# gautam-sabnis/A-Divide-and-Conquer-Strategy-for-High-Dimensional-Bayesian-Factor-Models

Measured on AMD Instinct MI355X. Metric: Gibbs iters/sec (node) at p=20k,n=1k,g=64; cov-assembly MFMA util %, higher is better.
Workload: dtype f64; 1 GPU; c3: p=19968 (P=312 x g=64), n=1000, K=30 (k=1920), rho=0.5, thin=5, burnin=0 (assembly in timed region), asm_batch=96; global_batch=1000, parallelism=shards64/gpus1

## Files before the change

a-divide-and-conquer-strategy-for-high-dimensional-bayesian-factor-models_amd/csrc/dcfm.hip:

```cpp
#include "handle.h"
#include "resid.h"

static int dalloc(dcfm_handle *h, double **p, size_t n) {
    void *q = nullptr;
    if (n == 0) n = 1;
    hipError_t e = hipMalloc(&q, n * sizeof(double));
    if (e != hipSuccess)
        return fail(h, DCFM_ERR_ALLOC, "hipMalloc(%zu doubles) failed: %s", n, hipGetErrorString(e));
    e = hipMemset(q, 0, n * sizeof(double));
    if (e != hipSuccess) return fail(h, DCFM_ERR_HIP, "hipMemset failed: %s", hipGetErrorString(e));
    h->allocs.push_back(q);
    *p = static_cast<double *>(q);
    return DCFM_OK;
}

static int round_up(int a, int b) { return (a + b - 1) / b * b; }

static double *trace_row(dcfm_handle *h, int64_t t) {
    return h->trace + trace_scratch_doubles(h->d.G) + (size_t)t * h->d.G * 4;
}

static void collect_prof(dcfm_handle *h) {
    if (h->recs.empty()) return;
    sync_all(h);
// ... 353 lines not shown
    if (h->d.inject) {
        if (!h->dr.NZ) return fail(h, DCFM_ERR_INVALID, "INJECT_DRAWS set but no draws");
        if (first_iter < h->dr.first_iter || first_iter + n_iter > h->dr.first_iter + h->dr.n_iter)
            return fail(h, DCFM_ERR_INVALID, "iterations [%lld,%lld) not covered by injected draws",
                        (long long)first_iter, (long long)(first_iter + n_iter));
    }
    return DCFM_OK;
}

struct DeltaTau { const double *delta_in, *tau_in; double *delta_out, *tau_out; };
static DeltaTau delta_tau(const dcfm_handle *h) {
    const size_t nkg = (size_t)h->d.g * h->d.kp, in = h->cur * nkg, out = (1 - h->cur) * nkg;
    return {h->b.delta + in, h->b.tau + in, h->b.delta + out, h->b.tau + out};
}

static void iteration_done(dcfm_handle *h) {
    h->cur ^= 1;
    if (h->trace_n < h->trace_cap) {
        launch_trace(h->d, h->b, delta_tau(h).tau_in, h->trace, trace_row(h, h->trace_n), h->stream);
        h->trace_n += 1;
    }
}

static void loading_rows(dcfm_handle *h, const DrawsDev &dr, int64_t it, bool lamgen) {
    const Dims &d = h->d;
    const Bufs &b = h->b;
    hipStream_t s = h->stream;
    const bool exact = h->cfg.flags & DCFM_FLAG_EXACT_RESIDUAL;
    const double kappa_max = exact ? HUGE_VAL : (h->cfg.flags & DCFM_FLAG_GUARD_ALL) ? 0.0 : KAPPA_IDENTITY_MAX;
    {
        KTimer t(h, DCFM_K_LAMBDA, s);
        launch_lambda(d, b, dr, it, delta_tau(h).tau_in, h->plam_valid ? b.Plam : nullptr, s, lamgen, kappa_max);
    }
    if (exact) {
        KTimer t(h, DCFM_K_RESID, s);
        launch_resid(d, b, dr, it, s, lamgen);
    } else if (d.kp != KP) {
        KTimer t(h, DCFM_K_RESID, s);
        launch_resid_flagged(d, b, dr, it, s);
    }
    h->plam_valid = false;
}

static int save_sample(dcfm_handle *h, int64_t it) {
    if (it % h->cfg.thin != 0 || it <= h->cfg.burnin) return DCFM_OK;
    const Bufs &b = h->b;
    hipStream_t s = h->stream;
    if (h->batch == 0 && h->asm_pending[h->lb]) {
        HIPC(h, hipStreamWaitEvent(s, h->e_free[h->lb], 0));
        h->asm_pending[h->lb] = false;
    }
    {
        KTimer t(h, DCFM_K_SAVE, s);
        launch_save(h->d, b, b.Lb[h->lb], b.wsum[h->lb], h->batch, s, b.wslot[h->lb], h->B);
        if (h->probe_n < h->probe_cap) launch_probes(h->d, b, h->probes, h->probe_n++, s);
        if (h->prec_n < h->prec_cap) launch_precision(h->d, b, h->prec, h->prec_n++, s);
    }
    HIPC(h, hipGetLastError());
    h->batch += 1;
    h->saved += 1;
    if (h->batch == h->B) TRY(flush_batch(h));
    return DCFM_OK;
}

struct FusedSchedule {
    dcfm_handle *h;
    const Dims &d;
    const Bufs &b;
    hipStream_t s;
    bool delta_pending = false;
    const DrawsDev &draws() const { return d.inject ? h->dr : h->gen[0]; }

    int step(int64_t it) {
        const DrawsDev &dr = draws();
        const bool lamgen = !d.inject;
        { KTimer t(h, DCFM_K_WPASS, s); launch_wcol(d, b, dr, it, true, delta_pending, true, ++h->wc_ops, s, lamgen); }
        if (d.coll) {
            { KTimer t(h, DCFM_K_XRED, s); launch_xred(d, b, s); }
            KTimer t(h, DCFM_K_COMM, s);
            TRY(coll_allgather(h, CH_MAIN, b.sloc, b.msg_all, (size_t)d.xstride, s));
        }
        {
            KTimer t(h, DCFM_K_XDRAW, s);
            if (d.coll) launch_xdraw_mr(d, b, dr, it, ++h->xm_ops, s);
            else launch_xdraw(d, b, dr, it, s, true);
        }
        {
            KTimer t(h, DCFM_K_CPASS, s);
            const DeltaTau dt = delta_tau(h);
            if (delta_pending) launch_cpass(d, b, s, dr, dt.delta_in, dt.tau_in, dt.delta_out, dt.tau_out, it - 1);
            else launch_cpass(d, b, s);
        }
        HIPC(h, hipGetLastError());
        if (delta_pending) iteration_done(h);
        loading_rows(h, dr, it, lamgen);
        delta_pending = true;
        return DCFM_OK;
    }

    int tail(int64_t last_iter) {
        if (!delta_pending) return DCFM_OK;
        KTimer t(h, DCFM_K_DELTA, s);
        launch_wcol(d, b, h->dr, last_iter, false, true, false, 0, s);
        if (d.coll) TRY(coll_allgather(h, CH_MAIN, b.sloc, b.msg_all, (size_t)d.xstride, s));
        const DeltaTau dt = delta_tau(h);
        launch_delta(d, b, draws(), last_iter, dt.delta_in, dt.tau_in, dt.delta_out, dt.tau_out, s);
        HIPC(h, hipGetLastError());
        iteration_done(h);
        return DCFM_OK;
    }
};

struct DrawBatches {
    dcfm_handle *h;
    int64_t end_iter;
    int64_t batch0, batch_n = 0;
    int slot = -1;
    int generate(int64_t b0, int busy) {
// ... 59 lines not shown
        if (!d.inject) TRY(gen.acquire(it));
        const DrawsDev &dr = d.inject ? h->dr : h->gen[gen.slot];
        HIPC(h, hipStreamWaitEvent(ss, h->e_lam, 0));
        { KTimer t(h, DCFM_K_PREP, ss); launch_prep(d, b, ss); }
        HIPC(h, hipEventRecord(h->e_prep, ss));
        { KTimer t(h, DCFM_K_XCHOL, ss); launch_asum(d, b, ss); }
        if (d.coll) {
            KTimer t(h, DCFM_K_COMM, ss);
            TRY(coll_allgather(h, CH_SIDE, b.xa, b.xa_all, KW * KW, ss));
        }
        { KTimer t(h, DCFM_K_XCHOL, ss); launch_xchol(d, b, ss); }
        HIPC(h, hipEventRecord(h->e_xchol, ss));
        { KTimer t(h, DCFM_K_WPASS, s);  launch_wpass(d, b, s); }
        HIPC(h, hipStreamWaitEvent(s, h->e_prep, 0));
        { KTimer t(h, DCFM_K_ZDRAW, s);  launch_zdraw(d, b, dr, it, s); }
        { KTimer t(h, DCFM_K_XRED, s);   launch_xred(d, b, s); }
        if (d.coll) {
            KTimer t(h, DCFM_K_COMM, s);
            TRY(coll_allgather(h, CH_MAIN, b.xin, b.xall, (size_t)d.NP * KW, s));
        }
        HIPC(h, hipStreamWaitEvent(s, h->e_xchol, 0));
        { KTimer t(h, DCFM_K_XDRAW, s); launch_xdraw(d, b, dr, it, s, false); }
        { KTimer t(h, DCFM_K_CPASS, s); launch_cpass(d, b, s); }
        loading_rows(h, dr, it, false);
        HIPC(h, hipEventRecord(h->e_lam, s));
        { KTimer t(h, DCFM_K_COLSUM, s); launch_colsum(d, b, s); }
        if (d.coll) {
            KTimer t(h, DCFM_K_COMM, s);
            TRY(coll_allgather(h, CH_MAIN, b.sloc, b.sall, (size_t)d.G * KW, s));
        }
        {
            KTimer t(h, DCFM_K_DELTA, s);
            const DeltaTau dt = delta_tau(h);
            launch_delta(d, b, dr, it, dt.delta_in, dt.tau_in, dt.delta_out, dt.tau_out, s);
        }
        if (!d.inject) TRY(gen.release(it));
        iteration_done(h);
        return DCFM_OK;
    }
};

int dcfm_run(dcfm_handle *h, int64_t first_iter, int64_t n_iter) {
    TRY(check_run_args(h, first_iter, n_iter));
    HIPC(h, hipSetDevice(h->cfg.device));
    hipStream_t s = h->stream;
    const int64_t end_iter = first_iter + n_iter;
    FusedSchedule fused{h, h->d, h->b, s};
// ... 126 lines not shown
```

a-divide-and-conquer-strategy-for-high-dimensional-bayesian-factor-models_amd/csrc/dcfm_internal.h:

```cpp
#pragma once
#include <hip/hip_runtime.h>
#include <stdint.h>

namespace dcfm {

constexpr int KP = 32;
constexpr int KP_MAX = 128;
constexpr int padded_width(int K) { return K <= 32 ? 32 : (K <= 64 ? 64 : 128); }
constexpr int ASM_TILE = 128;
__host__ __device__ constexpr int etile(int nbw, int Kc, int I) { return Kc * nbw - Kc * (Kc - 1) / 2 + (I - Kc); }
__host__ __device__ constexpr int etile_index(int nbw, int R, int Cc) {
    return (2 * etile(nbw, R >> 4, Cc >> 4) + ((R & 15) >> 3)) * 128 + 2 * ((Cc & 15) + 16 * (R & 3)) +
           (((R & 15) >> 2) & 1);
}
constexpr int ASM_KC = 16;
inline int cdiv(int a, int b) { return (a + b - 1) / b; }

struct Dims {
    int n, P, g, K, G;
    int NP, PP;
    int shard0;
    int nranks, rank;
    int coll;
    int p;
    int kp;
    double rho, sr, s1r;
    double as_, bs, df, ad1, bd1, ad2, bd2;
    uint64_t seed;
    int inject;
    int sgap, xstride;
};

struct DrawsDev {
    const double *NZ, *NX, *NL, *Gpsi, *Gdelta, *Gps;
    int64_t first_iter, n_iter;
};

struct LamDraws { const double *NL, *Gpsi, *Gps; };
#ifndef DCFM_LAM_GEN_BLOCKS
#define DCFM_LAM_GEN_BLOCKS 160
#endif
constexpr int LAM_GEN_THREADS = 256, LAM_GEN_BLOCKS = DCFM_LAM_GEN_BLOCKS;
struct LamGen { double *NL, *Gpsi, *Gps; int n_ps, n_psi, n_all, b_total; };
inline int lam_gen_doubles(const Dims &d) { return 2 * d.G * d.P * d.K + d.G * d.P; }
inline LamGen lam_gen_plan(const Dims &d, double *base) {
    const int T = LAM_GEN_THREADS, GP = d.G * d.P;
    LamGen g;
    g.NL = base;
    g.Gpsi = base + (size_t)GP * d.K;
    g.Gps = base + 2 * (size_t)GP * d.K;
    g.n_ps = GP;
    g.n_psi = GP + GP * d.K;
    g.n_all = g.n_psi + GP * ((d.K + 1) / 2);
    const int full = (g.n_all + T - 1) / T;
    g.b_total = full < LAM_GEN_BLOCKS ? full : LAM_GEN_BLOCKS;
    return g;
}

struct Bufs {
    double *Y, *yy, *Lam, *omega, *ps, *psi, *Plam, *X, *Z, *delta, *tau;
    double *ldraw;
// ... 66 lines not shown
}
__host__ __device__ inline long long win_off(long long c, long long c0, long long R0, long long R1) {
    const long long na = (c < R0 ? c : R0) - c0;
    const long long b0 = c0 > R0 ? c0 : R0, b1 = c < R1 ? c : R1;
    return (na > 0 ? na : 0) * (R1 - R0) + (b1 > b0 ? b1 - b0 : 0) * R1;
}

void launch_prep(const Dims &d, const Bufs &b, hipStream_t s);
void launch_wpass(const Dims &d, const Bufs &b, hipStream_t s);
void launch_zdraw(const Dims &d, const Bufs &b, const DrawsDev &dr, int64_t iter, hipStream_t s);
void launch_xred(const Dims &d, const Bufs &b, hipStream_t s);
void launch_wcol(const Dims &d, const Bufs &b, const DrawsDev &dr, int64_t iter, bool ops, bool colsum, bool wpass,
                 unsigned long long ops_epoch, hipStream_t s, bool lamgen = false);
void launch_xdraw_mr(const Dims &d, const Bufs &b, const DrawsDev &dr, int64_t iter, unsigned long long xm_epoch,
                     hipStream_t s);
void launch_asum(const Dims &d, const Bufs &b, hipStream_t s);
void launch_xchol(const Dims &d, const Bufs &b, hipStream_t s);
void launch_xdraw(const Dims &d, const Bufs &b, const DrawsDev &dr, int64_t iter, hipStream_t s,
                  bool from_shards = false);
void launch_cpass(const Dims &d, const Bufs &b, hipStream_t s, const DrawsDev &dr = DrawsDev{},
                  const double *delta_in = nullptr, const double *tau_in = nullptr, double *delta_out = nullptr,
                  double *tau_out = nullptr, int64_t delta_iter = 0);
void launch_lambda(const Dims &d, const Bufs &b, const DrawsDev &dr, int64_t iter,
                   const double *tau_cur, const double *plam_src, hipStream_t s, bool gen, double kappa_max);
void launch_colsum(const Dims &d, const Bufs &b, hipStream_t s);
void launch_resid(const Dims &d, const Bufs &b, const DrawsDev &dr, int64_t iter, hipStream_t s, bool gen);
void launch_resid_flagged(const Dims &d, const Bufs &b, const DrawsDev &dr, int64_t iter, hipStream_t s);
void launch_delta(const Dims &d, const Bufs &b, const DrawsDev &dr, int64_t iter,
                  const double *delta_in, const double *tau_in, double *delta_out,
                  double *tau_out, hipStream_t s);
void launch_save(const Dims &d, const Bufs &b, double *Lb, double *wsum, int slot, hipStream_t s,
                 double *wslot = nullptr, int B = 0);
void launch_assemble(const Dims &d, const Bufs &b, const double *Lb, const double *wsum, int kext,
                     double inv_eff, hipStream_t s);
void launch_assemble_m2(const Dims &d, const Bufs &b, const double *Lb, const double *wslot, int nslots, int B,
                        double inv_eff, hipStream_t s);
void launch_sigma_pack(const double *S, const double *S2, int which, double rs, int p, int T0, int T1, int c0,
                       int nc, double *out, hipStream_t s);
void launch_sigma_unpack(const double *recv, int p, int c0, int nc, const int *Tb, const long long *base,
                         int nranks, double *out, hipStream_t s);
void launch_eta(const Dims &d, const Bufs &b, double *eta_out, hipStream_t s);
int sigma_err_splits(int p);
void launch_sigma_err(const double *S, int p, const double *U, int R, const double *sdiag, const double *v,
                      int T0, int T1, bool first, double *y, double *fro, double *tru, double *out,
                      hipStream_t s);
size_t sigma_apply_scratch(int T0, int T1, int nv);
void launch_sigma_apply(const double *S, int p, int T0, int T1, const double *V, int nv, double *scratch, double *Y,
// ... 28 lines not shown
```

a-divide-and-conquer-strategy-for-high-dimensional-bayesian-factor-models_amd/csrc/kernels.hip:

```cpp
#include "dcfm_internal.h"
#include "philox.h"
#include "linalg.h"
#include "handoff.h"
#include "wstamp.h"
#include "zx_ops.h"
#include "ypass.h"
#include "draws.h"
#include "zdraw.h"
#include "delta.h"
#include "lambda.h"

#include <algorithm>

namespace dcfm {

__global__ __launch_bounds__(256) void k_prep(Dims d, const double *__restrict__ Lam,
                                              const double *__restrict__ omega,
                                              double *__restrict__ A, double *__restrict__ ZM) {
    __shared__ double smem[PREP_SMEM];
    prep_shard(d, Lam, omega, A, ZM, blockIdx.x, smem);
}

template <int KW>
__global__ __launch_bounds__(256) void k_wpass(Dims d, const double *__restrict__ Y,
// ... 27 lines not shown
    const int e = blockIdx.x * 256 + threadIdx.x;
    const int kk = d.kp * d.kp;
    if (e >= kk) return;
    xa[e] = tree_sum(A + e, d.G, (size_t)kk);
}

__global__ __launch_bounds__(256) void k_xchol(Dims d, const double *__restrict__ xa_all,
                                               double *__restrict__ XM) {
    __shared__ double smem[XCHOL_SMEM];
    for (int e = threadIdx.x; e < KP * KP; e += 256) {
        xprec_store(d, smem, e, tree_sum(xa_all + e, d.nranks, (size_t)d.xstride));
    }
    __syncthreads();
    xchol_factor(d, XM, smem);
}

__device__ __forceinline__ void xdraw_chunks(int nsrc, int &nch, int &chunk) {
    chunk = 1;
    while (nsrc / chunk > 4 && (nsrc / chunk) % 2 == 0) chunk *= 2;
    nch = nsrc / chunk;
    if (nch > 4) { nch = 1; chunk = nsrc; }
}
constexpr int XD_ROWS = 4;
constexpr int XD_SMEM = (2 * KP * (KP + 1) + 4 * 4 * 64 * 2) > XCHOL_SMEM ? (2 * KP * (KP + 1) + 4 * 4 * 64 * 2)
                                                                          : XCHOL_SMEM;
__global__ __launch_bounds__(1024) void k_xdraw(Dims d, const double *__restrict__ src, int nsrc, size_t sstride,
                                                double *__restrict__ XM,
                                                double *__restrict__ X, DrawsDev dr, int64_t iter, int xroles,
                                                const double *__restrict__ xa, unsigned long long *xm_ctr,
                                                unsigned long long xm_target) {
    __shared__ double smem[XD_SMEM];
    int blk = blockIdx.x;
    if (xroles & 1) {
        if (blk == 0) {
            for (int e = threadIdx.x; e < KP * KP; e += 1024)
                xprec_store(d, smem, e, d.nranks > 1 ? tree_sum(xa + e, d.nranks, (size_t)d.xstride) : xa[e]);
            __syncthreads();
            xchol_factor<true>(d, XM, smem);
            signal_count(xm_ctr);
            return;
        }
        blk -= 1;
    }
    double (*Ms)[KP][KP + 1] = reinterpret_cast<double (*)[KP][KP + 1]>(smem);
    d2 (*part)[4][64] = reinterpret_cast<d2 (*)[4][64]>(smem + 2 * KP * (KP + 1));
    const int lane = threadIdx.x & 63, w = threadIdx.x >> 6, c = lane & 15, q = lane >> 4;
    const int tw = w & 3, sw = w >> 2;
    const int i0 = blk * XD_ROWS, i = i0 + c;
    const bool live = c < XD_ROWS && i < d.n;
    const size_t stride = sstride;
    int nch, chunk;
    xdraw_chunks(nsrc, nch, chunk);
    d2 sv[4], ev[4];
    if (w == 0 && d.inject) {
        const double *nx = dr.NX + ((size_t)(iter - dr.first_iter) * d.n + (live ? i : 0)) * d.K;
#pragma unroll
        for (int t = 0; t < 4; ++t) {
            const int kk = 8 * t + 2 * q;
            ev[t].x = (live && kk < d.K) ? nx[kk] : 0.0;
            ev[t].y = (live && kk + 1 < d.K) ? nx[kk + 1] : 0.0;
        }
    } else if (w == 0) {
        const Rng rng(d.seed);
#pragma unroll
        for (int t = 0; t < 4; ++t) {
            const int kk = 8 * t + 2 * q;
            double n0 = 0.0, n1 = 0.0;
            if (live && kk < d.K) rng.normal2(SITE_X, 0u, (uint32_t)i, (uint32_t)(4 * t + q), (uint32_t)iter, n0, n1);
            ev[t].x = n0;
            ev[t].y = (kk + 1 < d.K) ? n1 : 0.0;
        }
    }
    double xmv[2] = {0.0, 0.0};
    if (!(xroles & 1)) {
#pragma unroll
        for (int u = 0; u < 2; ++u) xmv[u] = XM[threadIdx.x + 1024 * u];
    }
    if (sw < nch) {
        if (chunk >= 2) {
            constexpr int NPART = 16 / XD_ROWS;
            const int np = (chunk & (chunk - 1)) ? 1 : (chunk < NPART ? chunk : NPART), per = chunk / np;
            const int rr = c % XD_ROWS, h = c / XD_ROWS;
            const bool rl = i0 + rr < d.n && h < np;
            const double *p = src + (size_t)(sw * chunk + (h < np ? h : 0) * per) * stride +
                              (size_t)(i0 + rr < d.n ? i0 + rr : i0) * KP + 8 * tw + 2 * q;
            d2 v = rl ? tree_sum_f<d2, 8, 10>(per, [&](int rk) { return *reinterpret_cast<const d2 *>(p + (size_t)rk * stride); })
                      : d2{0.0, 0.0};
            for (int o = 1; o < np; o <<= 1) {
                d2 u;
                u.x = __shfl_down(v.x, o * XD_ROWS, 16);
                u.y = __shfl_down(v.y, o * XD_ROWS, 16);
                v.x = v.x + u.x;
                v.y = v.y + u.y;
            }
            part[sw][tw][lane] = h == 0 ? v : d2{0.0, 0.0};
        } else {
            const double *p = src + (size_t)sw * chunk * stride + (size_t)(live ? i : i0) * KP + 8 * tw + 2 * q;
            part[sw][tw][lane] = live ? *reinterpret_cast<const d2 *>(p) : d2{0.0, 0.0};
        }
    }
    if (xroles & 1) {
        wait_count(xm_ctr, xm_target);
#pragma unroll
        for (int u = 0; u < 2; ++u) xmv[u] = ld_agent(XM + threadIdx.x + 1024 * u);
    }
#pragma unroll
    for (int u = 0; u < 2; ++u) {
        const int e = threadIdx.x + 1024 * u;
        const int mat = e / (KP * KP), rem = e % (KP * KP);
        Ms[mat][rem / KP][rem % KP] = xmv[u];
    }
    __syncthreads();
    if (w > 0) return;
#pragma unroll
    for (int t = 0; t < 4; ++t) {
        TreeSum<d2, 3> ts;
        for (int k = 0; k < nch; ++k) ts.push(part[k][t][lane]);
        sv[t] = ts.total();
    }
    d4 ax[2];
    ax[0] = ax[1] = d4{0.0, 0.0, 0.0, 0.0};
#pragma unroll
    for (int t = 0; t < 4; ++t)
#pragma unroll
        for (int e = 0; e < 2; ++e) {
            const int kk = 8 * t + 2 * q + e;
            const double se = e ? sv[t].y : sv[t].x, ee = e ? ev[t].y : ev[t].x;
#pragma unroll
            for (int mt = 0; mt < 2; ++mt) {
                ax[mt] = mfma16x16x4(Ms[0][16 * mt + c][kk], se, ax[mt]);
                ax[mt] = mfma16x16x4(Ms[1][16 * mt + c][kk], ee, ax[mt]);
            }
        }
    if (!live) return;
    double *Xr = X + (size_t)i * KP;
#pragma unroll
// ... 332 lines not shown
    da.delta_in = delta_in; da.tau_in = tau_in; da.delta_out = delta_out; da.tau_out = tau_out;
    da.iter = delta_iter;
    const int ndel = (delta_in && d.kp == KP) ? cdiv(d.g, CP_WAVES) : 0;
    switch (d.kp) {
    case 32:
        if (grid.x < 128)
            hipLaunchKernelGGL((k_cpass<32, true>), dim3(2 * grid.x + ndel), dim3(64 * CP_WAVES), 0, s, d, b.Y,
                               b.X, b.Z, b.C, b.E, dr, b.sall, da, ndel);
        else
            hipLaunchKernelGGL((k_cpass<32, false>), dim3(grid.x + ndel), dim3(64 * CP_WAVES), 0, s, d, b.Y, b.X,
                               b.Z, b.C, b.E, dr, b.sall, da, ndel);
        break;
    case 64:
        launch_eta(d, b, b.W, s);
        hipLaunchKernelGGL(k_cpass<64>, grid, dim3(256), 0, s, d, b.Y, b.W, b.Z, b.C, b.E, dr, b.sall, da, 0);
        break;
    default:
        launch_eta(d, b, b.W, s);
        hipLaunchKernelGGL(k_cpass<128>, grid, dim3(256), 0, s, d, b.Y, b.W, b.Z, b.C, b.E, dr, b.sall, da, 0);
        break;
    }
}
void launch_lambda(const Dims &d, const Bufs &b, const DrawsDev &dr, int64_t iter,
                   const double *tau_cur, const double *plam_src, hipStream_t s, bool gen, double kappa_max) {
    if (d.kp != KP) return wide::launch_lambda(d, b, dr, iter, tau_cur, plam_src, s, kappa_max);
    const LamDraws ld = lam_draws_at(d, b, dr, iter, gen);
    const dim3 grid(cdiv(d.P, LAM_ROWS), d.G);
#define LAUNCH_LAM(KE)                                                                                       \
    hipLaunchKernelGGL(k_lambda<KE>, grid, dim3(64), 0, s, d, b.C, b.E, b.yy, tau_cur, b.Lam, b.psi, plam_src, \
                       b.ps, b.omega, b.cpart, ld, b.Y, b.X, b.Z, kappa_max)
    if (d.K <= 8) LAUNCH_LAM(8);
    else if (d.K <= 16) LAUNCH_LAM(16);
    else if (d.K <= 20) LAUNCH_LAM(20);
    else if (d.K <= 24) LAUNCH_LAM(24);
    else if (d.K <= 30) LAUNCH_LAM(30);
    else LAUNCH_LAM(32);
#undef LAUNCH_LAM
}
void launch_colsum(const Dims &d, const Bufs &b, hipStream_t s) {
    const dim3 grid(d.G, d.kp / 32);
    switch (d.kp) {
    case 32: hipLaunchKernelGGL(k_colsum<32>, grid, dim3(256), 0, s, d, b.cpart, b.sloc); break;
    case 64: hipLaunchKernelGGL(k_colsum<64>, grid, dim3(256), 0, s, d, b.cpart, b.sloc); break;
    default: hipLaunchKernelGGL(k_colsum<128>, grid, dim3(256), 0, s, d, b.cpart, b.sloc); break;
    }
}
void launch_delta(const Dims &d, const Bufs &b, const DrawsDev &dr, int64_t iter,
                  const double *delta_in, const double *tau_in, double *delta_out, double *tau_out,
                  hipStream_t s) {
    if (d.kp != KP) return wide::launch_delta(d, b, dr, iter, delta_in, tau_in, delta_out, tau_out, s);
    hipLaunchKernelGGL(k_delta, dim3(d.g), dim3(64), 0, s, d, b.sall, delta_in, tau_in, delta_out,
                       tau_out, dr, iter);
}
// ... 51 lines not shown
```

a-divide-and-conquer-strategy-for-high-dimensional-bayesian-factor-models_amd/csrc/lambda.h:

```cpp
#pragma once
#include "dcfm_internal.h"
#include "philox.h"
#include "linalg.h"
#include "resid.h"

namespace dcfm {

#ifndef DCFM_LAM_ILP
#define DCFM_LAM_ILP 4
#endif
constexpr int LAM_ILP = DCFM_LAM_ILP;
__device__ __forceinline__ void lam_draws(const Dims &d, const LamGen &lg, int64_t iter, int gtid, int gthreads) {
    const Rng rng(d.seed);
    const uint32_t it = (uint32_t)iter;
    const int kp2 = (d.K + 1) / 2;
    for (int x = gtid; x < lg.n_ps; x += gthreads) {
        const int m = x / d.P, j = x - m * d.P;
        lg.Gps[x] = rng.gamma(d.as_ + 0.5 * d.n, SITE_PS, (uint32_t)(d.shard0 + m), (uint32_t)j, 0u, it);
    }
    const double sh = d.df * 0.5 + 0.5;
    const int npsi = lg.n_psi - lg.n_ps;
    if (sh == 1.0 || sh == 2.0) {
        for (int y0 = gtid; y0 < npsi; y0 += LAM_ILP * gthreads) {
            double u[LAM_ILP];
// ... 59 lines not shown

struct LamPiv { double i00, i11, l10, v0, v1, t10; };
__device__ __forceinline__ LamPiv lam_pivots(d2 pk, d2 pk1, d2 bb) {
    LamPiv p;
    const double a = pk.x, bq = pk1.x, c2 = pk1.y;
    p.i00 = rsqrt_f64(a);
    p.l10 = bq * p.i00;
    const double d11 = c2 - p.l10 * p.l10;
    p.i11 = rsqrt_f64(d11);
    p.v0 = bb.x * p.i00;
    p.v1 = (bb.y - p.l10 * p.v0) * p.i11;
    p.t10 = p.l10 * p.i11;
    return p;
}

template <int KE>
__global__ __launch_bounds__(64) __attribute__((amdgpu_waves_per_eu(2))) void k_lambda(Dims d, const double *__restrict__ C, const double *__restrict__ E,
                                               const double *__restrict__ yy, const double *__restrict__ tau_cur,
                                               double *__restrict__ Lam, double *__restrict__ psi,
                                               const double *__restrict__ plam_src, double *__restrict__ ps,
                                               double *__restrict__ omega, double *__restrict__ cpart,
                                               LamDraws ld, const double *__restrict__ Y,
                                               const double *__restrict__ X, const double *__restrict__ Z,
                                               double kappa_max) {
    static_assert(KE % 2 == 0 && KE >= 2 && KE <= KP, "even factor width");
    constexpr int NB = (KE + 7) / 8;
    constexpr int LSN = 2 * LAM_ROWS * (KP + 1) * 2, BSN = 2 * LAM_ROWS * (KP + 2), VSN = LAM_ROWS * (KP + 2);
    constexpr int EP = KP + 2;
    static_assert(KP * EP <= LSN + BSN, "E staging fits the image area");
    __shared__ __attribute__((aligned(16))) double SM[LSN + BSN + 2 * VSN + KP];
    double(*LS)[LAM_ROWS][KP + 1][2] = reinterpret_cast<double(*)[LAM_ROWS][KP + 1][2]>(SM);
    double(*BS)[LAM_ROWS][KP + 2] = reinterpret_cast<double(*)[LAM_ROWS][KP + 2]>(SM + LSN);
    double *Vs = SM + LSN + BSN, *Is = Vs + VSN;
    double *Dg = SM + LSN + BSN + 2 * VSN;
    double *Es = SM;
    const int m = blockIdx.y, mg = d.shard0 + m;
    const int lane = threadIdx.x, grp = lane >> 3, l = lane & 7;
    Vs += grp * (KP + 2);
    Is += grp * (KP + 2);
    const int j0 = blockIdx.x * LAM_ROWS;
    const int j = j0 + grp;
    const bool valid = j < d.P;
    const int jj = valid ? j : 0;
    const uint32_t rowoff = (uint32_t)(m * d.PP + jj) * KP, toff = (uint32_t)mg * KP;
    bool rv[4];
#pragma unroll
    for (int b = 0; b < 4; ++b) rv[b] = valid && l + 8 * b < d.K;
// ... 228 lines not shown
#pragma unroll
    for (int b = 0; b < NB; ++b) {
        const double e = Dg[l + 8 * b < KE ? l + 8 * b : 0];
        sabs = (rv[b] && e > 0.0) ? fma(fabs(x[b]), e * __builtin_amdgcn_rsq(e), sabs) : sabs;
    }
    cs = fmax(cs, dpp8_d<0xB1>(cs));
    cs = fmax(cs, dpp8_d<0x4E>(cs));
    cs = fmax(cs, dpp8_d<0x141>(cs));
    double mag = valid ? (fma(cs + 1.0, ww, px) + 2.0 * wva) * ipsj : 0.0;
    sabs = rowsum8(sabs);
    mag = rowsum8(mag);
    const double SS = yyj + contrib;
    const bool reject = ss_identity_reject(yyj, SS, mag, sabs, kappa_max);
    const bool exact = __any(valid && reject);
    if (valid) {
#pragma unroll
        for (int b = 0; b < 4; ++b) {
            const int r = l + 8 * b;
            const double ps_b = rv[b] ? (1.0 / (d.df * 0.5 + 0.5 * (x[b] * x[b] * tv[b]))) * G[b] : 0.0;
            Lam[rowoff + r] = x[b];
            cpart[rowoff + r] = ps_b * (x[b] * x[b]);
            if (rv[b]) psi[rowoff + r] = ps_b;
        }
    }
    if (exact) {
        double(*Lm)[KP + 1] = reinterpret_cast<double(*)[KP + 1]>(SM);
#pragma unroll
        for (int b = 0; b < 4; ++b) Lm[grp][l + 8 * b] = x[b];
        __builtin_amdgcn_wave_barrier();
        const int cc = lane & 15;
        const double gps_c = ld.Gps[(uint32_t)(m * d.P) + (j0 + cc < d.P && cc < LAM_ROWS ? j0 + cc : 0)];
        resid_rows8(d, Y, X, Z, Lm, gps_c, m, j0, lane, ps, omega);
    } else if (valid && l == 0) {
        ps_omega_store(d, SS, Gps, ps, omega, (uint32_t)(m * d.PP + j));
    }
}

}
```

a-divide-and-conquer-strategy-for-high-dimensional-bayesian-factor-models_amd/csrc/linalg.h:

```cpp
#pragma once
#include <hip/hip_runtime.h>
#include "dcfm_internal.h"
#include "philox.h"

#include <type_traits>
#include <utility>

namespace dcfm {

typedef double d4 __attribute__((ext_vector_type(4)));
typedef double d2 __attribute__((ext_vector_type(2)));

__device__ __forceinline__ d4 mfma16x16x4(double a, double b, d4 c) {
    return __builtin_amdgcn_mfma_f64_16x16x4f64(a, b, c, 0, 0, 0);
}
__device__ __forceinline__ d4 mfma16x16x4_na(double a, double b, d4 c) {
    return __builtin_amdgcn_mfma_f64_16x16x4f64(a, b, c, 0, 0, 1);
}

__device__ __forceinline__ double readlane_d(double x, int l) {
    const int lo = __builtin_amdgcn_readlane(__double2loint(x), l);
    const int hi = __builtin_amdgcn_readlane(__double2hiint(x), l);
    return __hiloint2double(hi, lo);
}
// ... 24 lines not shown
            if (open) {
                if ((i >> Q) & 1) {
                    v = s[Q] + v;
                } else {
                    s[Q] = v;
                    open = false;
                }
            }
        });
        ++i;
    }
    __device__ __forceinline__ T total() const {
        T acc{};
        bool have = false;
        static_for<L>([&](auto Q) {
            if ((i >> Q) & 1) {
                acc = have ? s[Q] + acc : s[Q];
                have = true;
            }
        });
        return acc;
    }
};
template <class T, int B = 8, int L = TREE_LEVELS, class F>
__device__ __forceinline__ T tree_sum_f(int n, F &&load) {
    TreeSum<T, L> ts;
    for (int k = 0; k < n; k += B) {
        T v[B];
        static_for<B>([&](auto U) { if (k + U < n) v[U] = load(k + U); });
        static_for<B>([&](auto U) { if (k + U < n) ts.push(v[U]); });
    }
    return ts.total();
}
__device__ __forceinline__ double tree_sum(const double *__restrict__ src, int n, size_t stride) {
    return tree_sum_f<double>(n, [&](int k) { return src[(size_t)k * stride]; });
}

__device__ __forceinline__ double rsqrt_f64(double x) {
    double y = __builtin_amdgcn_rsq(x);
#pragma unroll
    for (int it = 0; it < 2; ++it) {
        const double e = fma(-x * y, y, 1.0);
        y = fma(0.5 * y, e, y);
    }
    return y;
}
// ... 353 lines not shown
```

a-divide-and-conquer-strategy-for-high-dimensional-bayesian-factor-models_amd/csrc/resid.h:

```cpp
#pragma once
#include "dcfm_internal.h"
#include "linalg.h"

namespace dcfm {

__device__ __forceinline__ void ps_omega_store(const Dims &d, double SS, double Gps, double *ps, double *omega,
                                               size_t at) {
    const double psn = (1.0 / (d.bs + 0.5 * SS)) * Gps;
    ps[at] = psn;
    omega[at] = 1.0 / psn;
}

#ifndef DCFM_KAPPA_MAX
#define DCFM_KAPPA_MAX 1e3
#endif
constexpr double KAPPA_IDENTITY_MAX = DCFM_KAPPA_MAX;
__device__ __forceinline__ bool ss_identity_reject(double yy, double SS, double mag, double sabs, double kappa_max) {
    const double rt = 1.01 * (yy * __builtin_amdgcn_rsq(yy) + sabs);
    const double num = fmax(rt * rt, 1.01 * (yy + mag));
    return !(SS > 0.0 && num <= kappa_max * SS);
}

__device__ __forceinline__ d2 eta_pair(const Dims &d, d2 x, d2 z) {
    return d2{eta_of(d.sr, d.s1r, x.x, z.x), eta_of(d.sr, d.s1r, x.y, z.y)};
}
template <int NT, int NH, class EtaAt>
__device__ __forceinline__ void resid_chunk(const d4 (&y)[NH], EtaAt eta_at, const d2 (&lb)[NH][NT], int row0, int n,
                                            double (&ss)[NH]) {
    d4 acc[NH];
#pragma unroll
    for (int h = 0; h < NH; ++h) acc[h] = y[h];
#pragma unroll
    for (int t = 0; t < NT; ++t) {
// ... 2 lines not shown
        for (int h = 0; h < NH; ++h) acc[h] = mfma16x16x4_na(e.x, lb[h][t].x, acc[h]);
#pragma unroll
        for (int h = 0; h < NH; ++h) acc[h] = mfma16x16x4_na(e.y, lb[h][t].y, acc[h]);
    }
#pragma unroll
    for (int h = 0; h < NH; ++h)
#pragma unroll
        for (int v = 0; v < 4; ++v)
            ss[h] = (row0 + 4 * v < n) ? fma(acc[h][v], acc[h][v], ss[h]) : ss[h];
}
template <int NH>
__device__ __forceinline__ void resid_lanesum(double (&ss)[NH]) {
#pragma unroll
    for (int h = 0; h < NH; ++h) {
        ss[h] += xor16_d(ss[h]);
        ss[h] += xor32_d(ss[h]);
    }
}

constexpr int LAM_ROWS = 8;
__device__ __forceinline__ void resid_rows8(const Dims &d, const double *__restrict__ Y,
                                            const double *__restrict__ X, const double *__restrict__ Z,
                                            const double (*Lm)[KP + 1], double Gps_c, int m, int j0, int lane,
                                            double *__restrict__ ps, double *__restrict__ omega) {
    constexpr int NT = KP / 8;
    const int c = lane & 15, q = lane >> 4;
    const bool col = c < LAM_ROWS && j0 + c < d.P;
    d2 lb[1][NT];
#pragma unroll
    for (int t = 0; t < NT; ++t) {
        lb[0][t].x = col ? Lm[c][8 * t + 2 * q] : 0.0;
        lb[0][t].y = col ? Lm[c][8 * t + 2 * q + 1] : 0.0;
    }
    const double *Ym = Y + (size_t)m * d.NP * d.PP + (col ? j0 + c : 0);
    const double *Zm = Z + (size_t)m * d.NP * KP + 2 * q;
    double ss[1] = {0.0};
    for (int i0 = 0; i0 < d.NP; i0 += 16) {
        d4 y[1];
#pragma unroll
        for (int v = 0; v < 4; ++v) y[0][v] = col ? Ym[(size_t)(i0 + q + 4 * v) * d.PP] : 0.0;
        const double *xr = X + (size_t)(i0 + c) * KP + 2 * q, *zr = Zm + (size_t)(i0 + c) * KP;
        resid_chunk(y, [&](int t) {
            return eta_pair(d, *reinterpret_cast<const d2 *>(xr + 8 * t), *reinterpret_cast<const d2 *>(zr + 8 * t));
        }, lb, i0 + q, d.n, ss);
    }
    resid_lanesum(ss);
    if (q == 0 && col) ps_omega_store(d, ss[0], Gps_c, ps, omega, (uint32_t)(m * d.PP + j0 + c));
}

template <int KW>
__device__ __forceinline__ void resid_tile(const Dims &d, const double *__restrict__ Y, const double *__restrict__ X,
                                           const double *__restrict__ Z, const double *__restrict__ Lam,
                                           const double *__restrict__ Gps, double *__restrict__ ps,
                                           double *__restrict__ omega, int m, int j0, double (*red)[32]) {
    constexpr int NT = KW / 8;
    const int lane = threadIdx.x & 63, w = threadIdx.x >> 6, c = lane & 15, q = lane >> 4;
    const double *Ym = Y + (size_t)m * d.NP * d.PP;
    const double *Zm = Z + (size_t)m * d.NP * KW;
    d2 lb[2][NT];
#pragma unroll
    for (int h = 0; h < 2; ++h)
#pragma unroll
        for (int t = 0; t < NT; ++t)
            lb[h][t] = *reinterpret_cast<const d2 *>(Lam + ((size_t)m * d.PP + j0 + 16 * h + c) * KW + 8 * t + 2 * q);
    double ss[2] = {0.0, 0.0};
    const int nch = d.NP / 16;
    for (int ch = w; ch < nch; ch += 4) {
        const int i0 = 16 * ch;
        d4 y[2];
#pragma unroll
// ... 24 lines not shown
```

a-divide-and-conquer-strategy-for-high-dimensional-bayesian-factor-models_amd/csrc/ypass.h:

```cpp
#pragma once
#include "dcfm_internal.h"
#include "linalg.h"

namespace dcfm {

#ifndef DCFM_WP_RING
#define DCFM_WP_RING 3
#endif
constexpr int WP_RING = DCFM_WP_RING;
#ifndef DCFM_WP_RING_WIDE
#define DCFM_WP_RING_WIDE 4
#endif
constexpr int WP_RING_WIDE = DCFM_WP_RING_WIDE;
template <int KW, int MT, int R = (KW > KP ? WP_RING_WIDE : WP_RING), class Pre>
__device__ __forceinline__ void wpass_acc(const Dims &d, const double *__restrict__ Y, const double *__restrict__ Lam,
                                          const double *__restrict__ omega, int m, int i0, int kt, d4 (&acc)[MT][2],
                                          Pre &&pre) {
    const int lane = threadIdx.x & 63;
    const int r = lane & 15, q = lane >> 4;
    const double *Y0 = Y + ((size_t)m * d.NP + i0 + r) * d.PP + 2 * q;
    const double *Y1 = Y0 + (size_t)16 * (MT - 1) * d.PP;
    const double *L = Lam + (size_t)m * d.PP * KW + 32 * kt + 2 * r;
    const double *wp = omega + (size_t)m * d.PP + 2 * q;
#pragma unroll
    for (int a = 0; a < MT; ++a)
#pragma unroll
        for (int b = 0; b < 2; ++b) acc[a][b] = d4{0.0, 0.0, 0.0, 0.0};
    const int nch = d.PP >> 3;
    d2 y0[R], y1[R], ww[R], l0[R], l1[R];
    auto load = [&](int t, int k) {
        const int j = 8 * t;
        y0[k] = *reinterpret_cast<const d2 *>(Y0 + j);
        if (MT == 2) y1[k] = *reinterpret_cast<const d2 *>(Y1 + j);
        ww[k] = *reinterpret_cast<const d2 *>(wp + j);
        l0[k] = *reinterpret_cast<const d2 *>(L + (size_t)(j + 2 * q) * KW);
        l1[k] = *reinterpret_cast<const d2 *>(L + (size_t)(j + 2 * q + 1) * KW);
    };
    d4 acc2[MT][2];
#pragma unroll
    for (int a = 0; a < MT; ++a)
#pragma unroll
        for (int b = 0; b < 2; ++b) acc2[a][b] = d4{0.0, 0.0, 0.0, 0.0};
    auto mma = [&](int k) {
        const double b00 = ww[k].x * l0[k].x, b01 = ww[k].x * l0[k].y;
        const double b10 = ww[k].y * l1[k].x, b11 = ww[k].y * l1[k].y;
        acc[0][0] = mfma16x16x4(b00, y0[k].x, acc[0][0]);
        acc[0][1] = mfma16x16x4(b01, y0[k].x, acc[0][1]);
        if (MT == 2) {
            acc[MT - 1][0] = mfma16x16x4(b00, y1[k].x, acc[MT - 1][0]);
            acc[MT - 1][1] = mfma16x16x4(b01, y1[k].x, acc[MT - 1][1]);
        }
// ... 107 lines not shown
```

Measured before the change: 5639 iter/s.

## Fuse sample saving into lambda kernel, spread xdraw RNG, skip padded wpass rows

```diff
diff --git a/a-divide-and-conquer-strategy-for-high-dimensional-bayesian-factor-models_amd/csrc/dcfm.hip b/a-divide-and-conquer-strategy-for-high-dimensional-bayesian-factor-models_amd/csrc/dcfm.hip
--- a/a-divide-and-conquer-strategy-for-high-dimensional-bayesian-factor-models_amd/csrc/dcfm.hip
+++ b/a-divide-and-conquer-strategy-for-high-dimensional-bayesian-factor-models_amd/csrc/dcfm.hip
@@ -399,15 +399,38 @@
     }
 }
 
-static void loading_rows(dcfm_handle *h, const DrawsDev &dr, int64_t it, bool lamgen) {
+static bool saved_iteration(const dcfm_handle *h, int64_t it) { return it % h->cfg.thin == 0 && it > h->cfg.burnin; }
+
+#ifndef DCFM_LAM_SAVE
+#define DCFM_LAM_SAVE 1
+#endif
+static bool lambda_saves(const dcfm_handle *h) {
+    return DCFM_LAM_SAVE && h->d.kp == KP && !(h->cfg.flags & DCFM_FLAG_EXACT_RESIDUAL);
+}
+
+static int open_batch(dcfm_handle *h) {
+    if (h->batch == 0 && h->asm_pending[h->lb]) {
+        HIPC(h, hipStreamWaitEvent(h->stream, h->e_free[h->lb], 0));
+        h->asm_pending[h->lb] = false;
+    }
+    return DCFM_OK;
+}
+
+static int loading_rows(dcfm_handle *h, const DrawsDev &dr, int64_t it, bool lamgen) {
     const Dims &d = h->d;
     const Bufs &b = h->b;
     hipStream_t s = h->stream;
     const bool exact = h->cfg.flags & DCFM_FLAG_EXACT_RESIDUAL;
     const double kappa_max = exact ? HUGE_VAL : (h->cfg.flags & DCFM_FLAG_GUARD_ALL) ? 0.0 : KAPPA_IDENTITY_MAX;
+    SaveArgs sv;
+    if (lambda_saves(h) && saved_iteration(h, it)) {
+        TRY(open_batch(h));
+        sv.Lb = b.Lb[h->lb]; sv.wsum = b.wsum[h->lb]; sv.wslot = b.wslot[h->lb];
+        sv.LDB = b.LDB; sv.slot = h->batch; sv.B = h->B;
+    }
     {
         KTimer t(h, DCFM_K_LAMBDA, s);
-        launch_lambda(d, b, dr, it, delta_tau(h).tau_in, h->plam_valid ? b.Plam : nullptr, s, lamgen, kappa_max);
+        launch_lambda(d, b, dr, it, delta_tau(h).tau_in, h->plam_valid ? b.Plam : nullptr, s, lamgen, kappa_max, sv);
     }
     if (exact) {
         KTimer t(h, DCFM_K_RESID, s);
@@ -417,19 +440,18 @@
         launch_resid_flagged(d, b, dr, it, s);
     }
     h->plam_valid = false;
+    return DCFM_OK;
 }
 
 static int save_sample(dcfm_handle *h, int64_t it) {
-    if (it % h->cfg.thin != 0 || it <= h->cfg.burnin) return DCFM_OK;
+    if (!saved_iteration(h, it)) return DCFM_OK;
     const Bufs &b = h->b;
     hipStream_t s = h->stream;
-    if (h->batch == 0 && h->asm_pending[h->lb]) {
-        HIPC(h, hipStreamWaitEvent(s, h->e_free[h->lb], 0));
-        h->asm_pending[h->lb] = false;
-    }
-    {
+    const bool ksave = !lambda_saves(h);
+    if (ksave) TRY(open_batch(h));
+    if (ksave || h->probe_n < h->probe_cap || h->prec_n < h->prec_cap) {
         KTimer t(h, DCFM_K_SAVE, s);
-        launch_save(h->d, b, b.Lb[h->lb], b.wsum[h->lb], h->batch, s, b.wslot[h->lb], h->B);
+        if (ksave) launch_save(h->d, b, b.Lb[h->lb], b.wsum[h->lb], h->batch, s, b.wslot[h->lb], h->B);
         if (h->probe_n < h->probe_cap) launch_probes(h->d, b, h->probes, h->probe_n++, s);
         if (h->prec_n < h->prec_cap) launch_precision(h->d, b, h->prec, h->prec_n++, s);
     }
@@ -470,7 +492,7 @@
         }
         HIPC(h, hipGetLastError());
         if (delta_pending) iteration_done(h);
-        loading_rows(h, dr, it, lamgen);
+        TRY(loading_rows(h, dr, it, lamgen));
         delta_pending = true;
         return DCFM_OK;
     }
@@ -576,7 +598,7 @@
         HIPC(h, hipStreamWaitEvent(s, h->e_xchol, 0));
         { KTimer t(h, DCFM_K_XDRAW, s); launch_xdraw(d, b, dr, it, s, false); }
         { KTimer t(h, DCFM_K_CPASS, s); launch_cpass(d, b, s); }
-        loading_rows(h, dr, it, false);
+        TRY(loading_rows(h, dr, it, false));
         HIPC(h, hipEventRecord(h->e_lam, s));
         { KTimer t(h, DCFM_K_COLSUM, s); launch_colsum(d, b, s); }
         if (d.coll) {
diff --git a/a-divide-and-conquer-strategy-for-high-dimensional-bayesian-factor-models_amd/csrc/dcfm_internal.h b/a-divide-and-conquer-strategy-for-high-dimensional-bayesian-factor-models_amd/csrc/dcfm_internal.h
--- a/a-divide-and-conquer-strategy-for-high-dimensional-bayesian-factor-models_amd/csrc/dcfm_internal.h
+++ b/a-divide-and-conquer-strategy-for-high-dimensional-bayesian-factor-models_amd/csrc/dcfm_internal.h
@@ -37,6 +37,10 @@
 };
 
 struct LamDraws { const double *NL, *Gpsi, *Gps; };
+struct SaveArgs {
+    double *Lb = nullptr, *wsum = nullptr, *wslot = nullptr;
+    int LDB = 0, slot = 0, B = 0;
+};
 #ifndef DCFM_LAM_GEN_BLOCKS
 #define DCFM_LAM_GEN_BLOCKS 160
 #endif
@@ -149,7 +153,8 @@
                   const double *delta_in = nullptr, const double *tau_in = nullptr, double *delta_out = nullptr,
                   double *tau_out = nullptr, int64_t delta_iter = 0);
 void launch_lambda(const Dims &d, const Bufs &b, const DrawsDev &dr, int64_t iter,
-                   const double *tau_cur, const double *plam_src, hipStream_t s, bool gen, double kappa_max);
+                   const double *tau_cur, const double *plam_src, hipStream_t s, bool gen, double kappa_max,
+                   const SaveArgs &sv = SaveArgs{});
 void launch_colsum(const Dims &d, const Bufs &b, hipStream_t s);
 void launch_resid(const Dims &d, const Bufs &b, const DrawsDev &dr, int64_t iter, hipStream_t s, bool gen);
 void launch_resid_flagged(const Dims &d, const Bufs &b, const DrawsDev &dr, int64_t iter, hipStream_t s);
diff --git a/a-divide-and-conquer-strategy-for-high-dimensional-bayesian-factor-models_amd/csrc/kernels.hip b/a-divide-and-conquer-strategy-for-high-dimensional-bayesian-factor-models_amd/csrc/kernels.hip
--- a/a-divide-and-conquer-strategy-for-high-dimensional-bayesian-factor-models_amd/csrc/kernels.hip
+++ b/a-divide-and-conquer-strategy-for-high-dimensional-bayesian-factor-models_amd/csrc/kernels.hip
@@ -73,8 +73,12 @@
     if (nch > 4) { nch = 1; chunk = nsrc; }
 }
 constexpr int XD_ROWS = 4;
-constexpr int XD_SMEM = (2 * KP * (KP + 1) + 4 * 4 * 64 * 2) > XCHOL_SMEM ? (2 * KP * (KP + 1) + 4 * 4 * 64 * 2)
-                                                                          : XCHOL_SMEM;
+#ifndef DCFM_XD_SPREAD
+#define DCFM_XD_SPREAD 1
+#endif
+constexpr bool XD_SPREAD = DCFM_XD_SPREAD;
+constexpr int XD_LDS = 2 * KP * (KP + 1) + 4 * 4 * 64 * 2 + 4 * 64 * 2;
+constexpr int XD_SMEM = XD_LDS > XCHOL_SMEM ? XD_LDS : XCHOL_SMEM;
 __global__ __launch_bounds__(1024) void k_xdraw(Dims d, const double *__restrict__ src, int nsrc, size_t sstride,
                                                 double *__restrict__ XM,
                                                 double *__restrict__ X, DrawsDev dr, int64_t iter, int xroles,
@@ -95,6 +99,7 @@
     }
     double (*Ms)[KP][KP + 1] = reinterpret_cast<double (*)[KP][KP + 1]>(smem);
     d2 (*part)[4][64] = reinterpret_cast<d2 (*)[4][64]>(smem + 2 * KP * (KP + 1));
+    d2 (*evs)[64] = reinterpret_cast<d2 (*)[64]>(smem + 2 * KP * (KP + 1) + 4 * 4 * 64 * 2);
     const int lane = threadIdx.x & 63, w = threadIdx.x >> 6, c = lane & 15, q = lane >> 4;
     const int tw = w & 3, sw = w >> 2;
     const int i0 = blk * XD_ROWS, i = i0 + c;
@@ -111,7 +116,7 @@
             ev[t].x = (live && kk < d.K) ? nx[kk] : 0.0;
             ev[t].y = (live && kk + 1 < d.K) ? nx[kk + 1] : 0.0;
         }
-    } else if (w == 0) {
+    } else if (w == 0 && !XD_SPREAD) {
         const Rng rng(d.seed);
 #pragma unroll
         for (int t = 0; t < 4; ++t) {
@@ -127,6 +132,13 @@
 #pragma unroll
         for (int u = 0; u < 2; ++u) xmv[u] = XM[threadIdx.x + 1024 * u];
     }
+    auto draw = [&] {
+        if (!XD_SPREAD || d.inject || w >= 4) return;
+        const int kk = 8 * w + 2 * q;
+        double n0 = 0.0, n1 = 0.0;
+        if (live && kk < d.K) Rng(d.seed).normal2(SITE_X, 0u, (uint32_t)i, (uint32_t)(4 * w + q), (uint32_t)iter, n0, n1);
+        evs[w][lane] = d2{n0, (kk + 1 < d.K) ? n1 : 0.0};
+    };
     if (sw < nch) {
         if (chunk >= 2) {
             constexpr int NPART = 16 / XD_ROWS;
@@ -135,8 +147,9 @@
             const bool rl = i0 + rr < d.n && h < np;
             const double *p = src + (size_t)(sw * chunk + (h < np ? h : 0) * per) * stride +
                               (size_t)(i0 + rr < d.n ? i0 + rr : i0) * KP + 8 * tw + 2 * q;
-            d2 v = rl ? tree_sum_f<d2, 8, 10>(per, [&](int rk) { return *reinterpret_cast<const d2 *>(p + (size_t)rk * stride); })
-                      : d2{0.0, 0.0};
+            d2 v = tree_sum_f<d2, 8, 10>(per, [&](int rk) {
+                return rl ? *reinterpret_cast<const d2 *>(p + (size_t)rk * stride) : d2{0.0, 0.0};
+            }, draw);
             for (int o = 1; o < np; o <<= 1) {
                 d2 u;
                 u.x = __shfl_down(v.x, o * XD_ROWS, 16);
@@ -147,7 +160,9 @@
             part[sw][tw][lane] = h == 0 ? v : d2{0.0, 0.0};
         } else {
             const double *p = src + (size_t)sw * chunk * stride + (size_t)(live ? i : i0) * KP + 8 * tw + 2 * q;
-            part[sw][tw][lane] = live ? *reinterpret_cast<const d2 *>(p) : d2{0.0, 0.0};
+            const d2 v = live ? *reinterpret_cast<const d2 *>(p) : d2{0.0, 0.0};
+            draw();
+            part[sw][tw][lane] = v;
         }
     }
     if (xroles & 1) {
@@ -163,6 +178,10 @@
     }
     __syncthreads();
     if (w > 0) return;
+    if (XD_SPREAD && !d.inject) {
+#pragma unroll
+        for (int t = 0; t < 4; ++t) ev[t] = evs[t][lane];
+    }
 #pragma unroll
     for (int t = 0; t < 4; ++t) {
         TreeSum<d2, 3> ts;
@@ -541,13 +560,14 @@
     }
 }
 void launch_lambda(const Dims &d, const Bufs &b, const DrawsDev &dr, int64_t iter,
-                   const double *tau_cur, const double *plam_src, hipStream_t s, bool gen, double kappa_max) {
+                   const double *tau_cur, const double *plam_src, hipStream_t s, bool gen, double kappa_max,
+                   const SaveArgs &sv) {
     if (d.kp != KP) return wide::launch_lambda(d, b, dr, iter, tau_cur, plam_src, s, kappa_max);
     const LamDraws ld = lam_draws_at(d, b, dr, iter, gen);
     const dim3 grid(cdiv(d.P, LAM_ROWS), d.G);
 #define LAUNCH_LAM(KE)                                                                                       \
     hipLaunchKernelGGL(k_lambda<KE>, grid, dim3(64), 0, s, d, b.C, b.E, b.yy, tau_cur, b.Lam, b.psi, plam_src, \
-                       b.ps, b.omega, b.cpart, ld, b.Y, b.X, b.Z, kappa_max)
+                       b.ps, b.omega, b.cpart, ld, b.Y, b.X, b.Z, kappa_max, sv)
     if (d.K <= 8) LAUNCH_LAM(8);
     else if (d.K <= 16) LAUNCH_LAM(16);
     else if (d.K <= 20) LAUNCH_LAM(20);
diff --git a/a-divide-and-conquer-strategy-for-high-dimensional-bayesian-factor-models_amd/csrc/lambda.h b/a-divide-and-conquer-strategy-for-high-dimensional-bayesian-factor-models_amd/csrc/lambda.h
--- a/a-divide-and-conquer-strategy-for-high-dimensional-bayesian-factor-models_amd/csrc/lambda.h
+++ b/a-divide-and-conquer-strategy-for-high-dimensional-bayesian-factor-models_amd/csrc/lambda.h
@@ -105,7 +105,7 @@
                                                double *__restrict__ omega, double *__restrict__ cpart,
                                                LamDraws ld, const double *__restrict__ Y,
                                                const double *__restrict__ X, const double *__restrict__ Z,
-                                               double kappa_max) {
+                                               double kappa_max, SaveArgs sv) {
     static_assert(KE % 2 == 0 && KE >= 2 && KE <= KP, "even factor width");
     constexpr int NB = (KE + 7) / 8;
     constexpr int LSN = 2 * LAM_ROWS * (KP + 1) * 2, BSN = 2 * LAM_ROWS * (KP + 2), VSN = LAM_ROWS * (KP + 2);
@@ -380,6 +380,12 @@
             cpart[rowoff + r] = ps_b * (x[b] * x[b]);
             if (rv[b]) psi[rowoff + r] = ps_b;
         }
+        if (sv.Lb) {
+            double *Lr = sv.Lb + ((size_t)mg * d.P + j) * sv.LDB + (size_t)sv.slot * d.K;
+#pragma unroll
+            for (int b = 0; b < 4; ++b)
+                if (rv[b]) Lr[l + 8 * b] = x[b];
+        }
     }
     if (exact) {
         double(*Lm)[KP + 1] = reinterpret_cast<double(*)[KP + 1]>(SM);
@@ -388,10 +394,10 @@
         __builtin_amdgcn_wave_barrier();
         const int cc = lane & 15;
         const double gps_c = ld.Gps[(uint32_t)(m * d.P) + (j0 + cc < d.P && cc < LAM_ROWS ? j0 + cc : 0)];
-        resid_rows8(d, Y, X, Z, Lm, gps_c, m, j0, lane, ps, omega);
+        resid_rows8(d, Y, X, Z, Lm, gps_c, m, j0, lane, ps, omega, sv);
     } else if (valid && l == 0) {
-        ps_omega_store(d, SS, Gps, ps, omega, (uint32_t)(m * d.PP + j));
-    }
-}
-
-}
+        ps_omega_store(d, SS, Gps, ps, omega, (uint32_t)(m * d.PP + j), sv, (size_t)mg * d.P + j);
+    }
+}
+
+}
diff --git a/a-divide-and-conquer-strategy-for-high-dimensional-bayesian-factor-models_amd/csrc/linalg.h b/a-divide-and-conquer-strategy-for-high-dimensional-bayesian-factor-models_amd/csrc/linalg.h
--- a/a-divide-and-conquer-strategy-for-high-dimensional-bayesian-factor-models_amd/csrc/linalg.h
+++ b/a-divide-and-conquer-strategy-for-high-dimensional-bayesian-factor-models_amd/csrc/linalg.h
@@ -70,6 +70,17 @@
         return acc;
     }
 };
+template <class T, int B = 8, int L = TREE_LEVELS, class F, class Mid>
+__device__ __forceinline__ T tree_sum_f(int n, F &&load, Mid &&mid) {
+    TreeSum<T, L> ts;
+    for (int k = 0; k == 0 || k < n; k += B) {
+        T v[B];
+        static_for<B>([&](auto U) { if (k + U < n) v[U] = load(k + U); });
+        if (k == 0) mid();
+        static_for<B>([&](auto U) { if (k + U < n) ts.push(v[U]); });
+    }
+    return ts.total();
+}
 template <class T, int B = 8, int L = TREE_LEVELS, class F>
 __device__ __forceinline__ T tree_sum_f(int n, F &&load) {
     TreeSum<T, L> ts;
diff --git a/a-divide-and-conquer-strategy-for-high-dimensional-bayesian-factor-models_amd/csrc/resid.h b/a-divide-and-conquer-strategy-for-high-dimensional-bayesian-factor-models_amd/csrc/resid.h
--- a/a-divide-and-conquer-strategy-for-high-dimensional-bayesian-factor-models_amd/csrc/resid.h
+++ b/a-divide-and-conquer-strategy-for-high-dimensional-bayesian-factor-models_amd/csrc/resid.h
@@ -9,6 +9,17 @@
     const double psn = (1.0 / (d.bs + 0.5 * SS)) * Gps;
     ps[at] = psn;
     omega[at] = 1.0 / psn;
+}
+__device__ __forceinline__ void ps_omega_store(const Dims &d, double SS, double Gps, double *ps, double *omega,
+                                               size_t at, const SaveArgs &sv, size_t a) {
+    const double psn = (1.0 / (d.bs + 0.5 * SS)) * Gps;
+    const double w = 1.0 / psn;
+    ps[at] = psn;
+    omega[at] = w;
+    if (sv.Lb) {
+        sv.wsum[a] += w;
+        if (sv.wslot) sv.wslot[a * sv.B + sv.slot] = w;
+    }
 }
 
 #ifndef DCFM_KAPPA_MAX
@@ -57,7 +68,7 @@
 __device__ __forceinline__ void resid_rows8(const Dims &d, const double *__restrict__ Y,
                                             const double *__restrict__ X, const double *__restrict__ Z,
                                             const double (*Lm)[KP + 1], double Gps_c, int m, int j0, int lane,
-                                            double *__restrict__ ps, double *__restrict__ omega) {
+                                            double *__restrict__ ps, double *__restrict__ omega, const SaveArgs &sv) {
     constexpr int NT = KP / 8;
     const int c = lane & 15, q = lane >> 4;
     const bool col = c < LAM_ROWS && j0 + c < d.P;
@@ -80,7 +91,8 @@
         }, lb, i0 + q, d.n, ss);
     }
     resid_lanesum(ss);
-    if (q == 0 && col) ps_omega_store(d, ss[0], Gps_c, ps, omega, (uint32_t)(m * d.PP + j0 + c));
+    if (q == 0 && col)
+        ps_omega_store(d, ss[0], Gps_c, ps, omega, (uint32_t)(m * d.PP + j0 + c), sv, (size_t)(d.shard0 + m) * d.P + j0 + c);
 }
 
 template <int KW>
diff --git a/a-divide-and-conquer-strategy-for-high-dimensional-bayesian-factor-models_amd/csrc/ypass.h b/a-divide-and-conquer-strategy-for-high-dimensional-bayesian-factor-models_amd/csrc/ypass.h
--- a/a-divide-and-conquer-strategy-for-high-dimensional-bayesian-factor-models_amd/csrc/ypass.h
+++ b/a-divide-and-conquer-strategy-for-high-dimensional-bayesian-factor-models_amd/csrc/ypass.h
@@ -12,6 +12,10 @@
 #define DCFM_WP_RING_WIDE 4
 #endif
 constexpr int WP_RING_WIDE = DCFM_WP_RING_WIDE;
+#ifndef DCFM_WP_SKIP_PAD
+#define DCFM_WP_SKIP_PAD 1
+#endif
+constexpr bool WP_SKIP_PAD = DCFM_WP_SKIP_PAD;
 template <int KW, int MT, int R = (KW > KP ? WP_RING_WIDE : WP_RING), class Pre>
 __device__ __forceinline__ void wpass_acc(const Dims &d, const double *__restrict__ Y, const double *__restrict__ Lam,
                                           const double *__restrict__ omega, int m, int i0, int kt, d4 (&acc)[MT][2],
@@ -26,7 +30,7 @@
     for (int a = 0; a < MT; ++a)
 #pragma unroll
         for (int b = 0; b < 2; ++b) acc[a][b] = d4{0.0, 0.0, 0.0, 0.0};
-    const int nch = d.PP >> 3;
+    const int nch = WP_SKIP_PAD ? (d.P + 7) >> 3 : d.PP >> 3;
     d2 y0[R], y1[R], ww[R], l0[R], l1[R];
     auto load = [&](int t, int k) {
         const int j = 8 * t;
```

New measurement: 5719 iter/s (median of 6 runs). 1.4% higher.
